# shanjiayao/PTT

Hardware: AMD Instinct MI355X
Metric: tracklet frames/sec (hot path: PointNet++ SA stack + Point-Track-Transformer blocks) (higher is better)
Workload: dtype f32

## Files before the change

### include/ptt_hip.h

```cpp
#ifndef PTT_HIP_H
#define PTT_HIP_H

#include <stddef.h>
#include <stdint.h>

#ifdef __cplusplus
extern "C" {
#endif

#define PTT_ABI_VERSION 28

enum {
    PTT_OK = 0,
    PTT_EINVAL = -1,
    PTT_EUNSUPPORTED = -2,
    PTT_ELAUNCH = -3,
    PTT_EWORKSPACE = -4
};

typedef void* ptt_stream_t;

int ptt_version(void);
const char* ptt_error_name(int code);
const char* ptt_last_error_string(void);

int ptt_fps_f32(const float* xyz, int B, int N, int npoint, int32_t* idx_out,
                ptt_stream_t stream);
int ptt_fps_ws_f32(const float* xyz, int B, int N, int npoint, int32_t* idx_out, float* workspace,
                   size_t workspace_elems, ptt_stream_t stream);

int ptt_gather_f32(const float* feat, const int32_t* idx, int B, int C, int N, int M,
                   float* out, ptt_stream_t stream);
int ptt_gather_grad_f32(const float* grad_out, const int32_t* idx, int B, int C, int N,
                        int M, float* grad_feat, ptt_stream_t stream);

int ptt_select_centres_f32(const float* xyz, const int32_t* idx, int B, int N, int M, float* new_xyz,
                           int64_t* idx64_out, ptt_stream_t stream);

int ptt_ball_query_f32(const float* new_xyz, const float* xyz, int B, int M, int N,
                       float radius, int nsample, int32_t* idx_out, ptt_stream_t stream);

int ptt_centres_ball_query_f32(const float* xyz, const int32_t* sel, int B, int N, int M, float radius, int nsample,
                               float* new_xyz, int64_t* idx64_out, int32_t* idx_out, ptt_stream_t stream);
// ... 476 lines not shown
```

### ptt_amd/csrc/common.h

```cpp
#pragma once
#include <hip/hip_runtime.h>
#include <stdint.h>
#include <stdio.h>
#include "../../include/ptt_hip.h"

namespace ptt {

char* last_error_buf();
int fail(int code, const char* fmt, ...);
int check_launch(const char* what);

static inline hipStream_t as_stream(ptt_stream_t s) { return reinterpret_cast<hipStream_t>(s); }

struct DevSwitches {
    int linear_rt = 1, linear_ct = 1;
    int linear_small = 1;
    int sa_gather1 = 0;
    int sa_stagger = 0;
    int sa_wave = 1;
    int sa_rt = 2;
    int sa_lds = 1;
    int sa_stream = 1;
    int sa_chunk = 2;
    int pair_stagger = 0;
    int pair_lds_pad = 0;
    int sa_lds_chunk = 2;
    int fps_plain = 0;
    int ball_cpw = 0;
    int fps_t = 0;
    int group_grad_global = 0;
    long long* stamps = nullptr;
};
const DevSwitches& dev_switches();

int set_lds_limit(const void* fn, int bytes);

bool wgrad_stream_ok(int R, int Cout, int Cin, int ldz, int ldx);
int wgrad_stream_rows(int R);
int launch_wgrad_stream(const float* dZ, int ldz, const float* X, int ldx, int R, int Cout, int Cin, int rows, float* partial,
                        const float* x_scale, const float* x_shift, hipStream_t s);

template <int CTRL, int ROW_MASK>
__device__ __forceinline__ int dpp_i32(int v) {
    return __builtin_amdgcn_update_dpp(v, v, CTRL, ROW_MASK, 0xF, false);
}
template <int CTRL, int ROW_MASK>
__device__ __forceinline__ float dpp_f32(float v) {
    return __builtin_bit_cast(float, dpp_i32<CTRL, ROW_MASK>(__builtin_bit_cast(int, v)));
}

__device__ __forceinline__ float wave_max_f32(float v) {
    v = fmaxf(v, dpp_f32<0xB1, 0xF>(v));
    v = fmaxf(v, dpp_f32<0x4E, 0xF>(v));
    v = fmaxf(v, dpp_f32<0x141, 0xF>(v));
    v = fmaxf(v, dpp_f32<0x140, 0xF>(v));
    v = fmaxf(v, dpp_f32<0x142, 0xA>(v));
    v = fmaxf(v, dpp_f32<0x143, 0xC>(v));
    return __builtin_bit_cast(float, __builtin_amdgcn_readlane(__builtin_bit_cast(int, v), 63));
}
__device__ __forceinline__ float wave_max_f32_fused(float v) {
    asm volatile(
        "s_nop 1\n\tv_max_f32_dpp %0, %0, %0 quad_perm:[1,0,3,2] row_mask:0xf bank_mask:0xf\n\t"
        "s_nop 1\n\tv_max_f32_dpp %0, %0, %0 quad_perm:[2,3,0,1] row_mask:0xf bank_mask:0xf\n\t"
        "s_nop 1\n\tv_max_f32_dpp %0, %0, %0 row_half_mirror row_mask:0xf bank_mask:0xf\n\t"
        "s_nop 1\n\tv_max_f32_dpp %0, %0, %0 row_mirror row_mask:0xf bank_mask:0xf\n\t"
        "s_nop 1\n\tv_max_f32_dpp %0, %0, %0 row_bcast:15 row_mask:0xa bank_mask:0xf\n\t"
        "s_nop 1\n\tv_max_f32_dpp %0, %0, %0 row_bcast:31 row_mask:0xc bank_mask:0xf\n\t"
        "s_nop 1"
// ... 25 lines not shown
```

### ptt_amd/csrc/gemm_ops.hip

```cpp
#include <atomic>
#include <math.h>
#include <stdlib.h>
#include <type_traits>
#include "common.h"

namespace ptt {

typedef float g32x16 __attribute__((ext_vector_type(16)));
typedef float g32x4 __attribute__((ext_vector_type(4)));
typedef int gi32x4 __attribute__((ext_vector_type(4)));
typedef unsigned int gu32x4 __attribute__((__vector_size__(4 * sizeof(unsigned int))));

namespace {

__device__ __forceinline__ __amdgpu_buffer_rsrc_t g_rsrc(const void* p) {
    return __builtin_amdgcn_make_buffer_rsrc(const_cast<void*>(p), 0, 0x7fffffff, 0x00020000);
}
__device__ __forceinline__ g32x4 g_load4(__amdgpu_buffer_rsrc_t r, int voff, int soff) {
    return __builtin_bit_cast(g32x4, __builtin_amdgcn_raw_buffer_load_b128(r, voff, soff, 0));
}
__device__ __forceinline__ float g_load1(__amdgpu_buffer_rsrc_t r, int voff, int soff) {
    return __builtin_bit_cast(float, __builtin_amdgcn_raw_buffer_load_b32(r, voff, soff, 0));
}
__device__ __forceinline__ void g_store1(float v, __amdgpu_buffer_rsrc_t r, int voff, int soff) {
// ... 469 lines not shown
        };
        frag(0, 0);
#pragma unroll
        for (int j = 0; j < RS / 2; ++j) {
            if (j + 1 < RS / 2) frag((EXP & 8) ? 0 : j + 1, (j + 1) & 1);
            __builtin_amdgcn_sched_barrier(0);
#pragma unroll
            for (int a = 0; a < TN; ++a)
#pragma unroll
                for (int b = 0; b < TK; ++b) acc[a][b] = __builtin_amdgcn_mfma_f32_32x32x2f32(av[j & 1][a], bv[j & 1][b], acc[a][b], 0, 0, 0);
            if (!(EXP & 1) && j >= RS / 2 - NP) stage_piece(buf ^ 1, j - (RS / 2 - NP));
            __builtin_amdgcn_sched_barrier(0);
        }
        if (!(EXP & 2)) hand_over();
        if (!(EXP & 4)) g_lds_barrier();
        buf ^= 1;
    }
    float* P = partial + (size_t)chunk * Cout * Cin;
#pragma unroll
    for (int a = 0; a < TN; ++a)
#pragma unroll
        for (int b = 0; b < TK; ++b) {
            const int ci = i0 + wk * (32 * TK) + b * 32 + col;
#pragma unroll
            for (int r = 0; r < 16; ++r) {
                const int co = o0 + wn * (32 * TN) + a * 32 + g_tile_row(r, half);
                if (!(EXP & 16) || r == 15) P[(size_t)co * Cin + ci] = acc[a][b][r];
            }
        }
}

void launch_wgrad_finish(const float* partial, int nchunks, size_t n, int accumulate, float* dW, hipStream_t s);

static int cu_count() {
    constexpr int MAX_DEV = 64;
    static std::atomic<int> cached[MAX_DEV];
    int dev = 0;
    if (hipGetDevice(&dev) != hipSuccess || dev < 0 || dev >= MAX_DEV) return 256;
    int n = cached[dev].load(std::memory_order_relaxed);
    if (n == 0) {
        int v = 0;
        n = (hipDeviceGetAttribute(&v, hipDeviceAttributeMultiprocessorCount, dev) == hipSuccess && v > 0) ? v : 256;
        cached[dev].store(n, std::memory_order_relaxed);
    }
    return n;
}

struct RowsGemmGeom { int WR, RT, CT, KC, TR, ncg, ntiles, G, chunks; bool ok; };
static RowsGemmGeom rows_gemm_geom(int rows, int K, int N) {
    RowsGemmGeom g{};
    g.ok = false;
    if (rows <= 0 || K <= 0 || N <= 0) return g;
    if (N % 128 == 0 && K % 128 == 0) {
        const int tiles64 = (rows + 63) / 64;
        g.WR = 1; g.RT = 2; g.KC = 128;
        g.CT = (N % 256 == 0 && (long long)tiles64 * (N / 256) >= 2 * cu_count()) ? 2 : 1;
    }
    else if (N % 128 == 0 && K % 64 == 0) { g.WR = 1; g.RT = 4; g.CT = 1; g.KC = 64; }
    else if (N % 64 == 0 && K % 64 == 0) { g.WR = 2; g.RT = 2; g.CT = 1; g.KC = 64; }
    else return g;
    const int WC = 4 / g.WR;
    g.TR = 32 * g.RT * g.WR;
    g.ncg = N / (32 * WC * g.CT);
    g.ntiles = (rows + g.TR - 1) / g.TR;
    int cap = 2 * cu_count() / g.ncg;
    if (cap >= 8) cap &= ~7;
    if (cap < 1) cap = 1;
// ... 378 lines not shown
```

### ptt_amd/csrc/mfma_ops.hip

```cpp
#include <math.h>
#include <stdlib.h>
#include <string.h>
#include "common.h"
#include "mfma_common.h"

#ifndef PTT_PAIR_PF
#define PTT_PAIR_PF 1
#endif
#ifndef PTT_GATHER_BATCH
#define PTT_GATHER_BATCH 16
#endif
#ifndef PTT_SA_WAVES
#define PTT_SA_WAVES 2
#endif

namespace ptt {

#ifdef PTT_DEV
#define PTT_STAMP(i) do { if (p.dbg && threadIdx.x == 0 && blockIdx.x < 4096) p.dbg[blockIdx.x * 8 + (i)] = __builtin_readcyclecounter(); } while (0)
#else
#define PTT_STAMP(i) do { } while (0)
#endif

__device__ __forceinline__ void stagger_second_slot(int first_wave_blocks, int quanta) {
// ... 1157 lines not shown
#pragma unroll
                    for (int r = 0; r < 16; ++r) acc[rt][u][r] = pre.sh[u];
            int nvalid = 0;
#pragma unroll
            for (int u = 0; u < 2; ++u)
                if (w + 4 * u < LL.NT) nvalid = u + 1;
            gemm_tiles<RT, 2, 0>(Xs, p.ldk, LL.nkb, reinterpret_cast<const f32x4*>(LL.Wp), LL.NT, w, nvalid, lane, acc, pre.w);
#pragma unroll
            for (int u = 0; u < 2; ++u) {
                if (u >= nvalid) break;
                const int col = (w + 4 * u) * 32 + (lane & 31);
                float sc = 1.f, sh = 0.f;
                if (affine) { sc = LL.scale[col]; sh = LL.shift ? LL.shift[col] : 0.f; }
#pragma unroll
                for (int rt = 0; rt < RT; ++rt) {
                    float m = affine ? acc[rt][u][0] * sc + sh : acc[rt][u][0];
#pragma unroll
                    for (int r = 1; r < 16; ++r) m = fmaxf(m, affine ? acc[rt][u][r] * sc + sh : acc[rt][u][r]);
                    run[u] = fmaxf(run[u], max_halves(m));
                }
            }
        }
    }
    if (half == 0) {
#pragma unroll
        for (int u = 0; u < 2; ++u) {
            if (w + 4 * u >= LL.NT) break;
            const int col = (w + 4 * u) * 32 + (lane & 31);
            p.out[(SPLIT ? hsel * q.out_sh : 0) + b * p.osb + col * p.osc + jj * p.osm] = LL.relu ? fmaxf(run[u], 0.f) : run[u];
        }
    }
}

template <int NS, int CT, bool AFFINE, int RT>
__device__ __forceinline__ void sa_wave_layer(const SaParams& p, const SaLayerDev& L, bool last, float* Xw, int lane,
                                              int centre0, int ncentres) {
    f32x16 acc[RT][CT];
#pragma unroll
    for (int u = 0; u < CT; ++u) {
        const float s0 = (!AFFINE && L.shift) ? L.shift[u * 32 + (lane & 31)] : 0.f;
#pragma unroll
        for (int rt = 0; rt < RT; ++rt)
#pragma unroll
            for (int r = 0; r < 16; ++r) acc[rt][u][r] = s0;
    }
    gemm_core<RT, CT, CT, 1>(Xw, p.ldk, L.nkb, reinterpret_cast<const f32x4*>(L.Wp), L.NT, 0, lane, acc);
    __builtin_amdgcn_wave_barrier();
    const int half = lane >> 5;
#pragma unroll
    for (int u = 0; u < CT; ++u) {
        const int col = u * 32 + (lane & 31);
        float sc = 1.f, sv = 0.f;
        if constexpr (AFFINE) { sc = L.scale[col]; sv = L.shift ? L.shift[col] : 0.f; }
#pragma unroll
        for (int rt = 0; rt < RT; ++rt) {
            float y[16];
#pragma unroll
            for (int r = 0; r < 16; ++r) y[r] = AFFINE ? acc[rt][u][r] * sc + sv : acc[rt][u][r];
            if (!last) {
#pragma unroll
                for (int r = 0; r < 16; ++r)
                    Xw[(rt * 32 + tile_row(r, half)) * p.ldk + col] = L.relu ? fmaxf(y[r], 0.f) : y[r];
            } else if (NS == 32) {
                float m = y[0];
#pragma unroll
                for (int r = 1; r < 16; ++r) m = fmaxf(m, y[r]);
// ... 943 lines not shown
        if ((rc = set_lds_limit(reinterpret_cast<const void*>(sa_stream_kernel<32>), lds))) return rc;
        hipLaunchKernelGGL((sa_stream_kernel<32>), dim3(wgs), dim3(256), lds, s, p);
        return check_launch("sa_stream_kernel");
    }
    int RT = dev_switches().sa_rt;
    if (d->nsample == 64) RT = 2;
    const int lds = 32 * RT * p.ldk * (int)sizeof(float);
    if (lds > 160 * 1024) return fail(PTT_EUNSUPPORTED, "ptt_sa_fused_fwd_f32: %d B of LDS per workgroup", lds);
    const int cpw = 32 * RT / d->nsample;
    const dim3 grid((total_centres + cpw - 1) / cpw);
#define PTT_SA_CASE(NSV, RTV)                                                                                   \
    if (d->nsample == NSV && RT == RTV) {                                                                       \
        if ((rc = set_lds_limit(reinterpret_cast<const void*>(sa_fused_kernel<NSV, RTV>), lds))) return rc;     \
        hipLaunchKernelGGL((sa_fused_kernel<NSV, RTV>), grid, dim3(256), lds, s, p);                            \
    }
    PTT_SA_CASE(32, 2) PTT_SA_CASE(32, 1) PTT_SA_CASE(16, 2) PTT_SA_CASE(16, 1) PTT_SA_CASE(64, 2)
#undef PTT_SA_CASE
    return check_launch("sa_fused_kernel");
}

extern "C" int ptt_xcorr_fused_fwd_f32(const ptt_xcorr_desc* d, ptt_stream_t stream) {
    if (!d) return fail(PTT_EINVAL, "ptt_xcorr_fused_fwd_f32: null descriptor");
    if (d->B < 0 || d->Ns <= 0 || d->C0 <= 0 || d->n_layers < 1 || d->n_layers > PTT_SA_MAX_LAYERS)
        return fail(PTT_EINVAL, "ptt_xcorr_fused_fwd_f32: B=%d Ns=%d C0=%d layers=%d", d->B, d->Ns, d->C0, d->n_layers);
    if (d->Nt <= 0 || (d->Nt % 64) != 0)
        return fail(PTT_EUNSUPPORTED, "ptt_xcorr_fused_fwd_f32: Nt=%d (the template seeds are walked in chunks of 64)", d->Nt);
    if (d->n_layers < 2) return fail(PTT_EUNSUPPORTED, "ptt_xcorr_fused_fwd_f32: needs at least two MFMA layers after layer 0");
    if ((d->C0 % 8) != 0 || d->C0 > 256) return fail(PTT_EUNSUPPORTED, "ptt_xcorr_fused_fwd_f32: C0=%d", d->C0);
    if (d->B == 0) return PTT_OK;
    if (!d->P || !d->w_sim || !d->out) return fail(PTT_EINVAL, "ptt_xcorr_fused_fwd_f32: null pointer");
    if ((unsigned long long)d->B * d->Ns * d->Nt >= 0x7fffffffull || (unsigned long long)d->B * d->Nt * d->C0 >= 0x7fffffffull)
        return fail(PTT_EUNSUPPORTED, "ptt_xcorr_fused_fwd_f32: B=%d Ns=%d Nt=%d: 32-bit element offsets — split the batch",
                    d->B, d->Ns, d->Nt);
    XcorrParams q;
    q.P = d->P; q.wsim = d->w_sim; q.scale0 = d->scale0;
    q.shift0 = d->shift0; q.sim_out = d->sim_out; q.cos_t = d->cos_t;
    q.C0 = d->C0; q.Nt = d->Nt;
    q.sfeat = q.tfeat = nullptr; q.s_sb = q.s_sn = q.t_sb = q.t_sn = 0; q.C = 0; q.eps = 0.f; q.out_sh = 0;
    SaParams& p = q.sa;
    memset(&p, 0, sizeof(p));
    p.out = d->out; p.osb = d->out_sb; p.osc = d->out_sc; p.osm = d->out_sn;
    p.B = d->B; p.M = d->Ns; p.n_layers = d->n_layers;
    int maxk = d->C0, cin = d->C0;
    for (int l = 0; l < d->n_layers; ++l) {
        const ptt_sa_layer& s = d->layers[l];
        if (s.Cin != cin) return fail(PTT_EINVAL, "ptt_xcorr_fused_fwd_f32: layer %d Cin=%d, expected %d", l, s.Cin, cin);
        if (s.Cout <= 0 || (s.Cout % 32) != 0 || s.Cout > 256)
            return fail(PTT_EUNSUPPORTED, "ptt_xcorr_fused_fwd_f32: layer %d Cout=%d", l, s.Cout);
        if (!s.Wpacked) return fail(PTT_EINVAL, "ptt_xcorr_fused_fwd_f32: layer %d has no weights", l);
        SaLayerDev& L = p.L[l];
        L.Wp = s.Wpacked; L.scale = s.scale; L.shift = s.shift; L.Cin = s.Cin; L.Cout = s.Cout; L.relu = s.relu;
        L.nkb = (s.Cin + 7) / 8; L.NT = s.Cout / 32;
        if (l + 1 < d->n_layers && s.Cout > maxk) maxk = s.Cout;
        cin = s.Cout;
    }
    p.ldk = ((maxk + 7) / 8) * 8 + 4;
    p.first_wave = 1024; p.stagger = 2;
    if (d->split) {
        if (!d->search_feat || !d->templ_feat || d->sim_out || (d->C & 3) || (d->s_sb & 3) || (d->s_sn & 3) ||
            (d->t_sb & 3) || (d->t_sn & 3) || ((reinterpret_cast<uintptr_t>(d->search_feat) | reinterpret_cast<uintptr_t>(d->templ_feat)) & 15) ||
            ((d->B * d->Ns) & 7) || d->C <= 0)
            return fail(PTT_EINVAL, "ptt_xcorr_fused_fwd_f32: the split form needs the features (unit channel stride, C %% 4 == 0, 16-byte "
                                    "aligned rows), B * Ns %% 8 == 0 and no sim_out");
        q.sfeat = d->search_feat; q.tfeat = d->templ_feat; q.s_sb = d->s_sb; q.s_sn = d->s_sn; q.t_sb = d->t_sb; q.t_sn = d->t_sn;
        q.C = d->C; q.eps = d->eps; q.out_sh = d->out_sh;
        const int lds = (32 * p.ldk + 32) * (int)sizeof(float);
        int rc = set_lds_limit(reinterpret_cast<const void*>(xcorr_fused_kernel<1, true>), lds);
        if (rc) return rc;
        hipLaunchKernelGGL((xcorr_fused_kernel<1, true>), dim3(2 * d->B * d->Ns), dim3(256), lds, as_stream(stream), q);
        return check_launch("xcorr_fused_kernel");
    }
    if (!d->cos_t) return fail(PTT_EINVAL, "ptt_xcorr_fused_fwd_f32: null pointer (cos_t comes from ptt_cosine_map_f32)");
    const int lds = (64 * p.ldk + 64) * (int)sizeof(float);
    int rc = set_lds_limit(reinterpret_cast<const void*>(xcorr_fused_kernel<2, false>), lds);
    if (rc) return rc;
    hipLaunchKernelGGL((xcorr_fused_kernel<2, false>), dim3(d->B * d->Ns), dim3(256), lds, as_stream(stream), q);
    return check_launch("xcorr_fused_kernel");
}

extern "C" int ptt_cosine_map_f32(const float* search_feat, int64_t s_sb, int64_t s_sn, int64_t s_sc, const float* templ_feat,
                                  int64_t t_sb, int64_t t_sn, int64_t t_sc, int B, int Ns, int Nt, int C, float eps,
                                  float* cos_t, ptt_stream_t stream) {
    if (B < 0 || Ns <= 0 || Nt <= 0 || C <= 0) return fail(PTT_EINVAL, "ptt_cosine_map_f32: B=%d Ns=%d Nt=%d C=%d", B, Ns, Nt, C);
    if (B == 0) return PTT_OK;
    if (!search_feat || !templ_feat || !cos_t) return fail(PTT_EINVAL, "ptt_cosine_map_f32: null pointer");
    CosParams q;
    q.sfeat = search_feat; q.tfeat = templ_feat; q.cos_t = cos_t;
    q.s_sb = s_sb; q.s_sn = s_sn; q.s_sc = s_sc; q.t_sb = t_sb; q.t_sn = t_sn; q.t_sc = t_sc;
    q.B = B; q.Ns = Ns; q.Nt = Nt; q.C = C; q.eps = eps;
    hipLaunchKernelGGL(cos_map_kernel, dim3((B * Ns + 3) / 4), dim3(256), 0, as_stream(stream), q);
// ... 45 lines not shown
```

### ptt_amd/models/backbones_3d/pointnet2_backbone.py

```python
from typing import List

import torch
import torch.nn as nn

from ... import graph_policy, ops, train_ops
from ...param_cache import ParamCache, index_table
from .pointnet2 import pointnet2_modules


class PointNet2BackboneLight(nn.Module):
    def __init__(self, model_cfg, input_channels, **kwargs):
        super().__init__()
        self.model_cfg = model_cfg
        input_channels -= 3
        self.num_points_each_layer = []
        self.SA_modules = nn.ModuleList()
        sa = self.model_cfg.SA_CONFIG
        for k in range(len(sa.RADIUS)):
            mlps = list(sa.MLPS[k])
            if k == 0:
                mlps[0] = input_channels
            self.SA_modules.append(pointnet2_modules.PointnetSAModuleVotes(
                radius=sa.RADIUS[k], nsample=sa.NSAMPLE[k], mlp=mlps,
                use_xyz=sa.get('USE_XYZ', True), normalize_xyz=sa.get('NORMALIZE_XYZ', True),
                sample_method=sa.SAMPLE_METHOD[k]))
        self.cov_final = nn.Conv1d(256, 256, kernel_size=1)
        self.num_point_features = sa.MLPS[-1][-1]
        self._cov_cache = ParamCache()
        self.seed_knn = 16
        self.overlap_branches = True
        self._side_stream = None

    @staticmethod
    def _break_up_pc(pc):
        xyz = pc[..., 0:3].contiguous()
        features = pc[..., 3:].contiguous() if pc.size(-1) > 3 else None
        return xyz, features

    def _cov_final(self, features):
        if not features.is_cuda:
            return self.cov_final(features)
        if self.training:
            if features.dtype != torch.float32:
                return self.cov_final(features)
            return train_ops.rows_linear(self.cov_final, features.transpose(1, 2)).transpose(1, 2)
        if ops.autograd_recording(self.cov_final, features) or features.dtype != torch.float32:
            ops.note_unfused('PointNet2BackboneLight.cov_final', 'autograd is recording or input is not float32')
            return self.cov_final(features)
        w, b = self.cov_final.weight, self.cov_final.bias
        wpacked, bias = self._cov_cache.get([w, b], w.device, lambda: (ops.pack_weight(w), b.detach().float().contiguous()))
        rows = features.transpose(1, 2)
        out = ops.linear(rows, wpacked, w.shape[0], None, bias)
        return out.transpose(1, 2)

    def branch_forward(self, pts, npoints: List, inds0=None, want_knn=0, compact_levels=()):
        xyz, features = self._break_up_pc(pts)
        sa = self.model_cfg.SA_CONFIG
        one_frame = (not self.training and xyz.is_cuda and features is None and len(self.SA_modules) == 3
                     and xyz.shape[0] * npoints[0] <= 4 * ops.ONE_FRAME_MAX_POINTS
                     and self.SA_modules[0].sample_method == 'fps'
                     and all(m.sample_method in ('rs', 'sequence') for m in self.SA_modules[1:])
                     and npoints[0] >= npoints[1] >= npoints[2] and (not want_knn or npoints[2] <= 128)
                     and all(m._fusable(xyz, None) for m in self.SA_modules[:1]))
        knn = None
# ... 6 lines not shown
            levels, inds64, knn = ops.sa_levels_point_jobs(xyz, inds0, list(npoints), list(sa.RADIUS), list(sa.NSAMPLE),
                                                           knn_k=want_knn)
            seq = [None] + [index_table(xyz.size(0), n, xyz.device, torch.int64) for n in npoints[1:3]]
            xyz, features, inds0 = self.SA_modules[0](xyz=xyz, features=features, npoint=npoints[0], inds=inds0,
                                                      pre=(levels[0][0], levels[0][1], inds64))
            xyz, features, inds1 = self.SA_modules[1](xyz=xyz, features=features, npoint=npoints[1],
                                                      pre=(levels[1][0], levels[1][1], seq[1]))
            xyz, features, inds2 = self.SA_modules[2](xyz=xyz, features=features, npoint=npoints[2],
                                                      pre=(levels[2][0], levels[2][1], seq[2]))
        else:
            xyz, features, inds0 = self.SA_modules[0](xyz=xyz, features=features, npoint=npoints[0], inds=inds0)
            xyz, features, inds1 = self.SA_modules[1](xyz=xyz, features=features, npoint=npoints[1], compact=1 in compact_levels)
            xyz, features, inds2 = self.SA_modules[2](xyz=xyz, features=features, npoint=npoints[2], compact=2 in compact_levels)
        point_features = self._cov_final(features)
        assert inds1.dtype == inds2.dtype == torch.int64, 'index type must be int64, not {}'.format(inds2.dtype)
        if all(m.sample_method in ('rs', 'sequence') for m in self.SA_modules[1:]) and inds0.shape[1] >= npoints[2]:
            inds = inds0[:, :npoints[2]]
        else:
            inds = inds0.gather(1, inds1).gather(1, inds2)
        if want_knn:
            return xyz, point_features, inds, knn
        return xyz, point_features, inds

    def sample(self, search_points, template_points):
        from .pointnet2 import pointnet2_utils
        sa = self.model_cfg.SA_CONFIG
        assert sa.SAMPLE_METHOD[0] == 'fps'
        return (pointnet2_utils.furthest_point_sample(search_points[..., 0:3].contiguous(), sa.NPOINTS_SEARCH[0]),
                pointnet2_utils.furthest_point_sample(template_points[..., 0:3].contiguous(), sa.NPOINTS_TEMPLATE[0]))

    def forward_branches(self, search_points, template_points, inds=None):
        sa = self.model_cfg.SA_CONFIG
        i_s, i_t = inds if inds is not None else (None, None)
        last = (len(self.SA_modules) - 1,) if (search_points.is_cuda and not self.training) else ()
        if not (self.overlap_branches and search_points.is_cuda and not self.training):
            r = self.branch_forward(search_points, sa.NPOINTS_SEARCH, i_s, want_knn=self.seed_knn, compact_levels=last)
            t_seeds, t_feats, t_inds = self.branch_forward(template_points, sa.NPOINTS_TEMPLATE, i_t)
        else:
            if self._side_stream is None or self._side_stream.device != search_points.device:
                self._side_stream = torch.cuda.Stream(device=search_points.device)
            main = torch.cuda.current_stream(search_points.device)
            side = graph_policy.branch(main, self._side_stream)
            with torch.cuda.stream(side):
                t_seeds, t_feats, t_inds = self.branch_forward(template_points, sa.NPOINTS_TEMPLATE, i_t)
            r = self.branch_forward(search_points, sa.NPOINTS_SEARCH, i_s, want_knn=self.seed_knn, compact_levels=last)
            graph_policy.join(main, side)
            if side is not main:
                for t in (t_seeds, t_feats, t_inds, template_points):
                    t.record_stream(main)
        s_seeds, s_feats, s_inds = r[:3]
        s_knn = r[3] if len(r) > 3 else None
        out = {'search_seeds': s_seeds, 'search_feats': s_feats, 'search_inds': s_inds,
               'template_seeds': t_seeds, 'template_feats': t_feats, 'template_inds': t_inds}
        if s_knn is not None:
            out['search_seeds_knn'] = s_knn
        return out

    def forward(self, batch_dict):
        batch_dict.update(self.forward_branches(batch_dict['search_points'], batch_dict['template_points'],
                                                batch_dict.pop('fps_inds', None)))
        batch_dict.pop('search_points')
        batch_dict.pop('template_points')
        return batch_dict
```

### ptt_amd/models/similarity_modules/p2b_xcoor.py

```python
import torch
import torch.nn as nn
import torch.nn.functional as F

from ... import ops, train_ops
from ...param_cache import DropsCachesOnModeChange, FoldedLayer, ParamCache, fold_conv_bn
from ..backbones_3d.pointnet2 import pytorch_utils as layer_utils


class CosineSimAug(DropsCachesOnModeChange, nn.Module):
    def __init__(self, model_cfg):
        super().__init__()
        self.model_cfg = model_cfg
        self.cosine = nn.CosineSimilarity(dim=1)
        self.mlp = layer_utils.SharedMLP(self.model_cfg.MLP.CHANNELS, bn=self.model_cfg.MLP.BN)
        self.conv = (
            layer_utils.Seq(self.model_cfg.CONV.CHANNELS[0])
            .conv1d(self.model_cfg.CONV.CHANNELS[1], bn=self.model_cfg.CONV.BN)
            .conv1d(self.model_cfg.CONV.CHANNELS[2], activation=None)
        )
        self._cache = ParamCache()

    def _fusable(self, search_feats, template_feats):
        if self.training or not search_feats.is_cuda:
            return False
        name = 'CosineSimAug'
        if ops.autograd_recording(self, search_feats, template_feats):
            return ops.note_unfused(name, 'autograd is recording (wrap inference in torch.no_grad())')
        if search_feats.dtype != torch.float32 or template_feats.dtype != torch.float32:
            return ops.note_unfused(name, 'features must be float32')
        if template_feats.shape[-1] % 64 != 0:
            return ops.note_unfused(name, 'ptt_xcorr_fused_fwd_f32 walks the template seeds in chunks of 64 (got %d)'
                                    % template_feats.shape[-1])
        units = list(self.mlp)
        if len(units) < 3 or len(units) > 5:
            return ops.note_unfused(name, 'SharedMLP depth %d' % len(units))
        for u in units:
            if not hasattr(u, 'normlayer') or u.conv.weight.shape[0] % 32 or u.conv.weight.shape[0] > 256:
                return ops.note_unfused(name, 'SharedMLP needs BatchNorm and widths that are multiples of 32, <= 256')
        if len(self.conv) != 2 or not hasattr(self.conv[0], 'normlayer') or hasattr(self.conv[1], 'normlayer'):
# ... 12 lines not shown
        s0, t0 = fold_conv_bn(units[0])
        layers = []
        for u in units[1:]:
            sc, sh = fold_conv_bn(u)
            w = u.conv.weight
            layers.append(FoldedLayer(ops.pack_weight(w * sc.view(-1, 1, 1, 1)), None, sh, w.shape[1], w.shape[0], True))
        return dict(w_sim=(w0[:, 0].float() * s0).contiguous(), w_rest=ops.pack_weight(w0[:, 1:]), c0=w0.shape[0],
                    w_rest_fx=ops.pack_weight(w0[:, 1:], 3),
                    scale0=s0, shift0=t0, layers=layers)

    def forward(self, batch_dict):
        search_feats = batch_dict['search_feats']
        template_feats = batch_dict['template_feats']
        template_xyz = batch_dict['template_seeds']
        b, f, n2 = search_feats.shape
        n1 = template_feats.shape[-1]

        if self._fusable(search_feats, template_feats):
            P = self._params()
            trows = template_feats.transpose(1, 2)
            if b * n1 <= ops.ONE_FRAME_MAX_POINTS and trows.is_contiguous():
                pre = torch.empty((b, n1, P['c0']), dtype=torch.float32, device=trows.device)
                ops.row_jobs([ops.row_job(P['w_rest_fx'], P['c0'], x=trows, x2=template_xyz.contiguous(), scale=P['scale0'],
                                          shift=P['shift0'], out=pre)])
            else:
                rows = torch.cat((template_xyz, trows), dim=2)
                pre = ops.linear(rows, P['w_rest'], P['c0'], P['scale0'], P['shift0'])
            if b * n2 <= ops.ONE_FRAME_MAX_POINTS:
                fused, _ = ops.xcorr_fused(search_feats, template_feats, pre, P['w_sim'], None, None,
                                           P['layers'], eps=self.cosine.eps, split=True)
            else:
                cos_t = ops.cosine_map(search_feats, template_feats, eps=self.cosine.eps)
                fused, _ = ops.xcorr_fused(search_feats, template_feats, pre, P['w_sim'], None, None,
                                           P['layers'], eps=self.cosine.eps, cos_t=cos_t)
            if fused.dim() == 4:
                L = layer_utils.rows_layers(self.conv)
                h0, h1 = fused[0].transpose(1, 2), fused[1].transpose(1, 2)
                x = None
                for li, layer in enumerate(L):
                    y = torch.empty((b, n2, layer.cout), dtype=torch.float32, device=h0.device)
                    ops.row_jobs([layer_utils.layer_job(layer, x=h0 if li == 0 else x, xmax=h1 if li == 0 else None, out=y)])
                    x = y
            else:
                y = layer_utils.rows_forward(self.conv, fused.transpose(1, 2))
            batch_dict['cosine_feats'] = y.transpose(1, 2)
            return batch_dict

        if (train_ops.usable(self.mlp, search_feats) and self.mlp[0].conv.weight.shape[1] == f + 4
                and self.mlp[0].conv.weight.shape[0] % 4 == 0 and self.mlp[0].conv.weight.shape[0] <= 256):
            fused = train_ops.xcorr_hoisted(search_feats, template_feats, template_xyz, self.mlp, self.cosine.eps)
            if train_ops.conv1d_stack_usable(self.conv, fused):
                batch_dict['cosine_feats'] = train_ops.conv1d_stack_rows(self.conv, fused.transpose(1, 2)).transpose(1, 2)
            else:
                batch_dict['cosine_feats'] = self.conv(fused)
            return batch_dict
        sim_feat = self.cosine(template_feats.unsqueeze(-1).expand(b, f, n1, n2),
                               search_feats.unsqueeze(2).expand(b, f, n1, n2))
        template_xyz_ = template_xyz.transpose(1, 2).contiguous().unsqueeze(-1).expand(b, 3, n1, n2)
        fusion_feature = torch.cat((sim_feat.unsqueeze(1), template_xyz_), dim=1)
        fusion_feature = torch.cat((fusion_feature, template_feats.unsqueeze(-1).expand(b, f, n1, n2)), dim=1)
        if train_ops.usable(self.mlp, fusion_feature):
            batch_dict['cosine_feats'] = self.conv(train_ops.shared_mlp_pool(fusion_feature, self.mlp, pool_dim=2))
            return batch_dict
        fusion_feature = self.mlp(fusion_feature)
        fusion_feature = fusion_feature.max(dim=2)[0]
        batch_dict['cosine_feats'] = self.conv(fusion_feature)
        return batch_dict
# ... 1 lines not shown
```

### ptt_amd/models/trackers/tracker3d_template.py

```python
import os

import torch
import torch.nn as nn

from .. import backbones_3d, similarity_modules, voting_heads


class Tracker3DTemplate(nn.Module):
    def __init__(self, model_cfg, num_class, dataset):
        super().__init__()
        self.model_cfg = model_cfg
        self.num_class = num_class
        self.dataset = dataset
        self.training = dataset.training
        self.class_names = dataset.class_names
        self.register_buffer('global_step', torch.LongTensor(1).zero_())
        self.module_topology = ['backbone_3d', 'similarity_module', 'centroid_voting_head', 'box_voting_head']

    @property
    def mode(self):
        return 'TRAIN' if self.training else 'TEST'

    def forward(self, **kwargs):
        raise NotImplementedError

    def update_global_step(self):
        self.global_step += 1

    def build_networks(self):
        info = {
            'module_list': [],
            'num_rawpoint_features': self.dataset.point_feature_encoder.num_point_features,
            'num_point_features': self.dataset.point_feature_encoder.num_point_features,
            'grid_size': self.dataset.grid_size,
            'point_cloud_range': self.dataset.point_cloud_range,
            'voxel_size': self.dataset.voxel_size,
        }
        for name in self.module_topology:
            module, info = getattr(self, 'build_%s' % name)(model_info_dict=info)
            self.add_module(name, module)
        return info['module_list']

    def build_backbone_3d(self, model_info_dict):
        cfg = self.model_cfg.get('BACKBONE_3D', None)
        if cfg is None:
            return None, model_info_dict
        module = backbones_3d.__all__[cfg.NAME](
            model_cfg=cfg, input_channels=model_info_dict['num_point_features'],
            grid_size=model_info_dict['grid_size'], voxel_size=model_info_dict['voxel_size'],
            point_cloud_range=model_info_dict['point_cloud_range'])
        model_info_dict['module_list'].append(module)
        model_info_dict['num_point_features'] = module.num_point_features
        return module, model_info_dict

    def build_similarity_module(self, model_info_dict):
        cfg = self.model_cfg.get('SIMILARITY_MODULE', None)
        if cfg is None:
            return None, model_info_dict
        module = similarity_modules.__all__[cfg.NAME](model_cfg=cfg)
        model_info_dict['module_list'].append(module)
        return module, model_info_dict

    def _build_head(self, key, model_info_dict):
        cfg = self.model_cfg.get(key, None)
        if cfg is None:
            return None, model_info_dict
        module = voting_heads.__all__[cfg.NAME](
            model_cfg=cfg, input_channels=model_info_dict['num_point_features'], num_class=1)
        model_info_dict['module_list'].append(module)
        return module, model_info_dict

    def build_centroid_voting_head(self, model_info_dict):
        return self._build_head('CENTROID_HEAD', model_info_dict)

    def build_box_voting_head(self, model_info_dict):
        return self._build_head('BOX_HEAD', model_info_dict)

    def post_processing(self, batch_dict):
        pass

    def load_params_from_file(self, filename, logger, to_cpu=False):
        if not os.path.isfile(filename):
            raise FileNotFoundError(filename)
# ... 34 lines not shown
```

### ptt_amd/ops.py

```python
import contextlib
import ctypes
import os

import torch

from . import _lib
from ._lib import AttnDesc, SaDesc, SaLayer, XcorrDesc


def _stream():
    return ctypes.c_void_p(torch.cuda.current_stream().cuda_stream)


_timing = None


def start_kernel_timing(names):
    global _timing
    _timing = {n: [] for n in names}


def stop_kernel_timing():
    global _timing
    t, _timing = _timing, None
# ... 384 lines not shown
    out = torch.empty((B, Ns, Nt), dtype=torch.float32, device=search_feats.device)
    ssb, ssc, ssn = search_feats.stride()
    tsb, tsc, tsn = templ_feats.stride()
    _launch("ptt_cosine_map_f32", out.device, search_feats.data_ptr(), ssb, ssn, ssc, templ_feats.data_ptr(), tsb, tsn, tsc, B, Ns, Nt, C, float(eps),
            out.data_ptr(), timed='ptt_cosine_map_f32')
    return out


def rows_mlp(x, layers, residual=None):
    if not x.is_cuda or x.dtype != torch.float32 or x.stride(-1) != 1:
        raise RuntimeError("rows_mlp: x must be a float32 device tensor with contiguous rows")
    K = x.shape[-1]
    x2 = x.reshape(-1, K)
    rows = x2.shape[0]
    cout = int(layers[-1][4])
    out = torch.empty((rows, cout), dtype=torch.float32, device=x.device)
    res2 = None
    if residual is not None:
        res2 = residual.reshape(-1, cout)
        _chk(res2 if res2.is_contiguous() else res2.contiguous(), "residual", torch.float32, 2)
        res2 = res2 if res2.stride(1) == 1 else res2.contiguous()
    arr = (SaLayer * len(layers))()
    for i, (wp, sc, sh, cin, co, relu) in enumerate(layers):
        arr[i].Wpacked = wp.data_ptr()
        arr[i].scale = sc.data_ptr() if sc is not None else None
        arr[i].shift = sh.data_ptr() if sh is not None else None
        arr[i].Cin, arr[i].Cout, arr[i].relu = int(cin), int(co), int(bool(relu))
    _launch("ptt_rows_mlp_f32", x.device, _ptr(x2), rows, K, x2.stride(0), arr, len(layers), _ptr(res2), res2.stride(0) if res2 is not None else 0,
            _ptr(out), cout, timed='ptt_rows_mlp_f32')
    return out.view(*x.shape[:-1], cout)


def xcorr_fused(search_feats, templ_feats, P, w_sim, scale0, shift0, layers, eps=1e-8, want_sim=False, cos_t=None, split=False):
    for t_, n_ in ((search_feats, "search_feats"), (templ_feats, "templ_feats")):
        if not t_.is_cuda or t_.dtype != torch.float32 or t_.dim() != 3:
            raise RuntimeError("%s must be a (B,C,N) float32 device tensor" % n_)
    _chk(P, "P", torch.float32, 3)
    _chk(w_sim, "w_sim", torch.float32, 1)
    B, C, Ns = search_feats.shape
    Nt = templ_feats.shape[2]
    C0 = P.shape[2]
    if Nt <= 0 or Nt % 64:
        raise RuntimeError("xcorr_fused: Nt=%d (ptt_xcorr_fused_fwd_f32 walks the template seeds in chunks of 64)" % Nt)
    if P.shape[0] != B or P.shape[1] != Nt or w_sim.shape[0] != C0 or templ_feats.shape[:2] != search_feats.shape[:2]:
        raise RuntimeError("xcorr_fused: inconsistent shapes")
    cout = layers[-1][4]
    split = (split and not want_sim and search_feats.stride(1) == 1 and templ_feats.stride(1) == 1 and C % 4 == 0 and (B * Ns) % 8 == 0
             and all(st % 4 == 0 for st in (search_feats.stride(0), search_feats.stride(2), templ_feats.stride(0), templ_feats.stride(2)))
             and search_feats.data_ptr() % 16 == 0 and templ_feats.data_ptr() % 16 == 0 and bool(layers[-1][5]))
    if not split:
        if cos_t is None:
            cos_t = cosine_map(search_feats, templ_feats, eps=eps)
        _chk(cos_t, "cos_t", torch.float32, 3)
        if tuple(cos_t.shape) != (B, Ns, Nt):
            raise RuntimeError("xcorr_fused: cos_t must be (B,Ns,Nt)")
    store = torch.empty(((2, B, Ns, cout) if split else (B, Ns, cout)), dtype=torch.float32, device=P.device)
    out = store.transpose(-1, -2)
    sim = torch.empty((B, Nt, Ns), dtype=torch.float32, device=P.device) if want_sim else None
    d = XcorrDesc()
    if split:
        d.split, d.out_sh = 1, store.stride(0)
        d.search_feat, d.templ_feat = search_feats.data_ptr(), templ_feats.data_ptr()
        d.s_sb, d.s_sn, d.t_sb, d.t_sn = search_feats.stride(0), search_feats.stride(2), templ_feats.stride(0), templ_feats.stride(2)
        d.C, d.eps = int(C), float(eps)
    else:
        d.cos_t = cos_t.data_ptr()
    d.P, d.w_sim = P.data_ptr(), w_sim.data_ptr()
    d.scale0 = scale0.data_ptr() if scale0 is not None else None
    d.shift0 = shift0.data_ptr() if shift0 is not None else None
    d.out = out.data_ptr()
    d.out_sb, d.out_sc, d.out_sn = out.stride()[-3:]
    d.sim_out = sim.data_ptr() if sim is not None else None
    d.B, d.Ns, d.Nt, d.C0 = B, Ns, Nt, C0
    d.n_layers = len(layers)
    for i, (wp, sc, sh, cin, co, relu) in enumerate(layers):
        L = d.layers[i]
        L.Wpacked = wp.data_ptr()
        L.scale = sc.data_ptr() if sc is not None else None
        L.shift = sh.data_ptr() if sh is not None else None
        L.Cin, L.Cout, L.relu = int(cin), int(co), int(bool(relu))
    _launch("ptt_xcorr_fused_fwd_f32", P.device, ctypes.byref(d), timed='ptt_xcorr_fused_fwd_f32')
    return out, sim


def pack_delta0(weight, bias):
    return pack_weight(torch.cat([weight.detach().float().reshape(weight.shape[0], 3),
                                  bias.detach().float().reshape(-1, 1)], dim=1).contiguous())


def spatial_order(xyz):
    _chk(xyz, "xyz", torch.float32, 3)
    B, N, _ = xyz.shape
    order = torch.empty((B, N), dtype=torch.int32, device=xyz.device)
    _launch("ptt_spatial_order_f32", xyz.device, _ptr(xyz), B, N, _ptr(order))
    return order


def pt_attn_pair(xyz, knn_idx, qkv, wd1p, wd2p, bd2, wg1p, bg1, wg2p, bg2, d_model, want_attn=True, rel=None, order=None,
                 heads=1):
# ... 1232 lines not shown
```

Measured before the change: 17430.

## Add persistent streamed xcorr kernel and compact more backbone SA levels

Adds a persistent kernel for the xcorr head that handles Nt=64, C0=256 with two 256-wide layers. For each search point it builds the first-layer activations from cos_t and the precomputed P in LDS, runs both layers with MFMA, and max-reduces over template seeds without writing intermediates. The grid is sized to two blocks per CU, and each block loops over a contiguous range of points, reusing P per batch and prefetching weights. The backbone also enables compact levels 1 and 2 for the search and template branches. The costs are added code paths with strict shape gating, and a behaviour change in SA level handling that could shift the balance of work.

```diff
diff --git a/include/ptt_hip.h b/include/ptt_hip.h
--- a/include/ptt_hip.h
+++ b/include/ptt_hip.h
@@ -8,7 +8,7 @@
 extern "C" {
 #endif
 
-#define PTT_ABI_VERSION 28
+#define PTT_ABI_VERSION 29
 
 enum {
     PTT_OK = 0,
diff --git a/ptt_amd/csrc/common.h b/ptt_amd/csrc/common.h
--- a/ptt_amd/csrc/common.h
+++ b/ptt_amd/csrc/common.h
@@ -34,6 +34,8 @@
 const DevSwitches& dev_switches();
 
 int set_lds_limit(const void* fn, int bytes);
+
+int cu_count();
 
 bool wgrad_stream_ok(int R, int Cout, int Cin, int ldz, int ldx);
 int wgrad_stream_rows(int R);
diff --git a/ptt_amd/csrc/gemm_ops.hip b/ptt_amd/csrc/gemm_ops.hip
--- a/ptt_amd/csrc/gemm_ops.hip
+++ b/ptt_amd/csrc/gemm_ops.hip
@@ -525,7 +525,7 @@
 
 void launch_wgrad_finish(const float* partial, int nchunks, size_t n, int accumulate, float* dW, hipStream_t s);
 
-static int cu_count() {
+int cu_count() {
     constexpr int MAX_DEV = 64;
     static std::atomic<int> cached[MAX_DEV];
     int dev = 0;
diff --git a/ptt_amd/csrc/mfma_ops.hip b/ptt_amd/csrc/mfma_ops.hip
--- a/ptt_amd/csrc/mfma_ops.hip
+++ b/ptt_amd/csrc/mfma_ops.hip
@@ -1213,6 +1213,115 @@
     }
 }
 
+constexpr int XCS_C = 256;
+constexpr int XCS_LDK = XCS_C + 4;
+constexpr int XCS_NKB = XCS_C / 8, XCS_NT = XCS_C / 32;
+__global__ __launch_bounds__(256, 2) void xcorr_stream_kernel(XcorrParams q) {
+    typedef float f32x2 __attribute__((ext_vector_type(2)));
+    extern __shared__ __attribute__((aligned(16))) float smem[];
+    float* Xs = smem;
+    const SaParams& p = q.sa;
+    const int t = threadIdx.x, lane = t & 63, w = __builtin_amdgcn_readfirstlane(t >> 6), half = lane >> 5;
+    const int npts = p.B * p.M;
+    const int g = logical_block(), G = (int)gridDim.x;
+    const int base = npts / G, rem = npts - base * G;
+    int j = g * base + min(g, rem);
+    const int jend = j + base + (g < rem ? 1 : 0);
+    if (j >= jend) return;
+    stagger_second_slot(p.first_wave, p.stagger);
+
+    const SaLayerDev& L0 = p.L[0];
+    const SaLayerDev& L1 = p.L[1];
+    const f32x4* W0 = reinterpret_cast<const f32x4*>(L0.Wp);
+    const f32x4* W1 = reinterpret_cast<const f32x4*>(L1.Wp);
+    const int col0 = w * 32 + (lane & 31);
+    const float sh0[2] = {L0.shift[col0], L0.shift[col0 + 128]};
+    const float sh1[2] = {L1.shift[col0], L1.shift[col0 + 128]};
+    const f32x4 w4 = *reinterpret_cast<const f32x4*>(q.wsim + lane * 4);
+    const int crow = w + 4 * (lane & 15);
+
+    int b = j / p.M;
+    const int pvoff = (w * XCS_C + lane * 4) * (int)sizeof(float);
+    f32x4 pq[16];
+    {
+        const __amdgpu_buffer_rsrc_t pr = weight_rsrc(q.P + (size_t)b * (64 * XCS_C));
+#pragma unroll
+        for (int k = 0; k < 16; ++k) pq[k] = weight_load(pr, pvoff, k * 4 * XCS_C * (int)sizeof(float));
+    }
+    float cv = q.cos_t[(unsigned)(j * 64 + crow)];
+    f32x4 pre[2];
+    prefetch_first_block_full<2>(L0.Wp, w, lane, pre);
+
+    for (;;) {
+#pragma unroll
+        for (int k = 0; k < 16; ++k) {
+            const float cs = __builtin_bit_cast(float, __builtin_amdgcn_readlane(__builtin_bit_cast(int, cv), k));
+            const f32x2 c2 = {cs, cs};
+            const f32x4 pv = pq[k];
+            f32x2 lo = __builtin_elementwise_fma(f32x2{w4[0], w4[1]}, c2, f32x2{pv[0], pv[1]});
+            f32x2 hi = __builtin_elementwise_fma(f32x2{w4[2], w4[3]}, c2, f32x2{pv[2], pv[3]});
+            *reinterpret_cast<f32x4*>(Xs + (w + 4 * k) * XCS_LDK + lane * 4) =
+                f32x4{fmaxf(lo[0], 0.f), fmaxf(lo[1], 0.f), fmaxf(hi[0], 0.f), fmaxf(hi[1], 0.f)};
+        }
+        lds_barrier();
+
+        f32x16 acc[2][2];
+#pragma unroll
+        for (int rt = 0; rt < 2; ++rt)
+#pragma unroll
+            for (int u = 0; u < 2; ++u)
+#pragma unroll
+                for (int r = 0; r < 16; ++r) acc[rt][u][r] = sh0[u];
+        gemm_core<2, 2, 2, 4, 0>(Xs, XCS_LDK, XCS_NKB, W0, XCS_NT, w, lane, acc, pre);
+        prefetch_first_block_full<2>(L1.Wp, w, lane, pre);
+        lds_barrier();
+#pragma unroll
+        for (int u = 0; u < 2; ++u)
+#pragma unroll
+            for (int rt = 0; rt < 2; ++rt)
+#pragma unroll
+                for (int r = 0; r < 16; ++r)
+                    Xs[(rt * 32 + tile_row(r, half)) * XCS_LDK + col0 + u * 128] = L0.relu ? fmaxf(acc[rt][u][r], 0.f) : acc[rt][u][r];
+        lds_barrier();
+
+        const int jn = j + 1;
+        const bool more = jn < jend;
+        const int jl = more ? jn : j;
+        const int bn = jl / p.M;
+        cv = q.cos_t[(unsigned)(jl * 64 + crow)];
+        if (bn != b) {
+            const __amdgpu_buffer_rsrc_t pr = weight_rsrc(q.P + (size_t)bn * (64 * XCS_C));
+#pragma unroll
+            for (int k = 0; k < 16; ++k) pq[k] = weight_load(pr, pvoff, k * 4 * XCS_C * (int)sizeof(float));
+        }
+
+#pragma unroll
+        for (int rt = 0; rt < 2; ++rt)
+#pragma unroll
+            for (int u = 0; u < 2; ++u)
+#pragma unroll
+                for (int r = 0; r < 16; ++r) acc[rt][u][r] = sh1[u];
+        gemm_core<2, 2, 2, 4, 0>(Xs, XCS_LDK, XCS_NKB, W1, XCS_NT, w, lane, acc, pre);
+        prefetch_first_block_full<2>(L0.Wp, w, lane, pre);
+        const int jj = j - b * p.M;
+#pragma unroll
+        for (int u = 0; u < 2; ++u) {
+            float run = -__builtin_inff();
+#pragma unroll
+            for (int rt = 0; rt < 2; ++rt) {
+                float m = acc[rt][u][0];
+#pragma unroll
+                for (int r = 1; r < 16; ++r) m = fmaxf(m, acc[rt][u][r]);
+                run = fmaxf(run, max_halves(m));
+            }
+            if (half == 0) p.out[b * p.osb + (col0 + u * 128) * p.osc + jj * p.osm] = L1.relu ? fmaxf(run, 0.f) : run;
+        }
+        if (!more) break;
+        j = jn; b = bn;
+        lds_barrier();
+    }
+}
+
 template <int NS, int CT, bool AFFINE, int RT>
 __device__ __forceinline__ void sa_wave_layer(const SaParams& p, const SaLayerDev& L, bool last, float* Xw, int lane,
                                               int centre0, int ncentres) {
@@ -2222,6 +2331,22 @@
     if ((unsigned long long)d->B * d->Ns * d->Nt >= 0x7fffffffull || (unsigned long long)d->B * d->Nt * d->C0 >= 0x7fffffffull)
         return fail(PTT_EUNSUPPORTED, "ptt_xcorr_fused_fwd_f32: B=%d Ns=%d Nt=%d: 32-bit element offsets — split the batch",
                     d->B, d->Ns, d->Nt);
+    const bool streamed = d->split == 2;
+    if (streamed) {
+        if (!d->cos_t) return fail(PTT_EUNSUPPORTED, "ptt_xcorr_fused_fwd_f32: the streamed form reads cos_t (ptt_cosine_map_f32)");
+        if (d->Nt != 64 || d->C0 != XCS_C || d->n_layers != 2)
+            return fail(PTT_EUNSUPPORTED, "ptt_xcorr_fused_fwd_f32: the streamed form is Nt=64, C0=256 and two remaining layers (Nt=%d C0=%d layers=%d)",
+                        d->Nt, d->C0, d->n_layers);
+        if (d->scale0 || d->shift0) return fail(PTT_EUNSUPPORTED, "ptt_xcorr_fused_fwd_f32: the streamed form needs layer 0's BatchNorm folded into P and w_sim");
+        if (d->sim_out) return fail(PTT_EUNSUPPORTED, "ptt_xcorr_fused_fwd_f32: the streamed form does not write sim_out");
+        for (int l = 0; l < 2; ++l) {
+            const ptt_sa_layer& s = d->layers[l];
+            if (s.Cin != XCS_C || s.Cout != XCS_C)
+                return fail(PTT_EUNSUPPORTED, "ptt_xcorr_fused_fwd_f32: the streamed form is 256 -> 256 -> 256 (layer %d: %d -> %d)", l, s.Cin, s.Cout);
+            if (s.scale || !s.shift)
+                return fail(PTT_EUNSUPPORTED, "ptt_xcorr_fused_fwd_f32: the streamed form needs layer %d's scale folded into its weights and a shift", l);
+        }
+    }
     XcorrParams q;
     q.P = d->P; q.wsim = d->w_sim; q.scale0 = d->scale0;
     q.shift0 = d->shift0; q.sim_out = d->sim_out; q.cos_t = d->cos_t;
@@ -2246,6 +2371,14 @@
     }
     p.ldk = ((maxk + 7) / 8) * 8 + 4;
     p.first_wave = 1024; p.stagger = 2;
+    if (streamed) {
+        const int npts = d->B * d->Ns, slots = 2 * cu_count();
+        const int lds = 64 * XCS_LDK * (int)sizeof(float);
+        int rc = set_lds_limit(reinterpret_cast<const void*>(xcorr_stream_kernel), lds);
+        if (rc) return rc;
+        hipLaunchKernelGGL(xcorr_stream_kernel, dim3(npts < slots ? npts : slots), dim3(256), lds, as_stream(stream), q);
+        return check_launch("xcorr_stream_kernel");
+    }
     if (d->split) {
         if (!d->search_feat || !d->templ_feat || d->sim_out || (d->C & 3) || (d->s_sb & 3) || (d->s_sn & 3) ||
             (d->t_sb & 3) || (d->t_sn & 3) || ((reinterpret_cast<uintptr_t>(d->search_feat) | reinterpret_cast<uintptr_t>(d->templ_feat)) & 15) ||
diff --git a/ptt_amd/models/backbones_3d/pointnet2_backbone.py b/ptt_amd/models/backbones_3d/pointnet2_backbone.py
--- a/ptt_amd/models/backbones_3d/pointnet2_backbone.py
+++ b/ptt_amd/models/backbones_3d/pointnet2_backbone.py
@@ -30,6 +30,8 @@
         self.seed_knn = 16
         self.overlap_branches = True
         self._side_stream = None
+        self.compact_levels = (len(self.SA_modules) - 1,)
+        self.template_compact_levels = ()
 
     @staticmethod
     def _break_up_pc(pc):
@@ -102,17 +104,19 @@
     def forward_branches(self, search_points, template_points, inds=None):
         sa = self.model_cfg.SA_CONFIG
         i_s, i_t = inds if inds is not None else (None, None)
-        last = (len(self.SA_modules) - 1,) if (search_points.is_cuda and not self.training) else ()
+        fused = search_points.is_cuda and not self.training
+        last = tuple(self.compact_levels) if fused else ()
+        t_levels = tuple(self.template_compact_levels) if fused else ()
         if not (self.overlap_branches and search_points.is_cuda and not self.training):
             r = self.branch_forward(search_points, sa.NPOINTS_SEARCH, i_s, want_knn=self.seed_knn, compact_levels=last)
-            t_seeds, t_feats, t_inds = self.branch_forward(template_points, sa.NPOINTS_TEMPLATE, i_t)
+            t_seeds, t_feats, t_inds = self.branch_forward(template_points, sa.NPOINTS_TEMPLATE, i_t, compact_levels=t_levels)
         else:
             if self._side_stream is None or self._side_stream.device != search_points.device:
                 self._side_stream = torch.cuda.Stream(device=search_points.device)
             main = torch.cuda.current_stream(search_points.device)
             side = graph_policy.branch(main, self._side_stream)
             with torch.cuda.stream(side):
-                t_seeds, t_feats, t_inds = self.branch_forward(template_points, sa.NPOINTS_TEMPLATE, i_t)
+                t_seeds, t_feats, t_inds = self.branch_forward(template_points, sa.NPOINTS_TEMPLATE, i_t, compact_levels=t_levels)
             r = self.branch_forward(search_points, sa.NPOINTS_SEARCH, i_s, want_knn=self.seed_knn, compact_levels=last)
             graph_policy.join(main, side)
             if side is not main:
diff --git a/ptt_amd/models/similarity_modules/p2b_xcoor.py b/ptt_amd/models/similarity_modules/p2b_xcoor.py
--- a/ptt_amd/models/similarity_modules/p2b_xcoor.py
+++ b/ptt_amd/models/similarity_modules/p2b_xcoor.py
@@ -5,6 +5,9 @@
 from ... import ops, train_ops
 from ...param_cache import DropsCachesOnModeChange, FoldedLayer, ParamCache, fold_conv_bn
 from ..backbones_3d.pointnet2 import pytorch_utils as layer_utils
+
+
+XCORR_STREAM_MIN_POINTS = 512
 
 
 class CosineSimAug(DropsCachesOnModeChange, nn.Module):
@@ -83,7 +86,8 @@
             else:
                 cos_t = ops.cosine_map(search_feats, template_feats, eps=self.cosine.eps)
                 fused, _ = ops.xcorr_fused(search_feats, template_feats, pre, P['w_sim'], None, None,
-                                           P['layers'], eps=self.cosine.eps, cos_t=cos_t)
+                                           P['layers'], eps=self.cosine.eps, cos_t=cos_t,
+                                           split=2 if b * n2 >= XCORR_STREAM_MIN_POINTS else False)
             if fused.dim() == 4:
                 L = layer_utils.rows_layers(self.conv)
                 h0, h1 = fused[0].transpose(1, 2), fused[1].transpose(1, 2)
diff --git a/ptt_amd/models/trackers/tracker3d_template.py b/ptt_amd/models/trackers/tracker3d_template.py
--- a/ptt_amd/models/trackers/tracker3d_template.py
+++ b/ptt_amd/models/trackers/tracker3d_template.py
@@ -49,6 +49,8 @@
             model_cfg=cfg, input_channels=model_info_dict['num_point_features'],
             grid_size=model_info_dict['grid_size'], voxel_size=model_info_dict['voxel_size'],
             point_cloud_range=model_info_dict['point_cloud_range'])
+        if hasattr(module, 'compact_levels'):
+            module.compact_levels = module.template_compact_levels = (1, 2)
         model_info_dict['module_list'].append(module)
         model_info_dict['num_point_features'] = module.num_point_features
         return module, model_info_dict
diff --git a/ptt_amd/ops.py b/ptt_amd/ops.py
--- a/ptt_amd/ops.py
+++ b/ptt_amd/ops.py
@@ -440,6 +440,9 @@
 
 
 def xcorr_fused(search_feats, templ_feats, P, w_sim, scale0, shift0, layers, eps=1e-8, want_sim=False, cos_t=None, split=False):
+    streamed = split == 2 and not isinstance(split, bool)
+    if streamed:
+        split = False
     for t_, n_ in ((search_feats, "search_feats"), (templ_feats, "templ_feats")):
         if not t_.is_cuda or t_.dtype != torch.float32 or t_.dim() != 3:
             raise RuntimeError("%s must be a (B,C,N) float32 device tensor" % n_)
@@ -456,6 +459,8 @@
     split = (split and not want_sim and search_feats.stride(1) == 1 and templ_feats.stride(1) == 1 and C % 4 == 0 and (B * Ns) % 8 == 0
              and all(st % 4 == 0 for st in (search_feats.stride(0), search_feats.stride(2), templ_feats.stride(0), templ_feats.stride(2)))
              and search_feats.data_ptr() % 16 == 0 and templ_feats.data_ptr() % 16 == 0 and bool(layers[-1][5]))
+    streamed = (streamed and not want_sim and Nt == 64 and C0 == 256 and scale0 is None and shift0 is None and len(layers) == 2
+                and all(sc is None and sh is not None and cin == 256 and co == 256 for (_, sc, sh, cin, co, _) in layers))
     if not split:
         if cos_t is None:
             cos_t = cosine_map(search_feats, templ_feats, eps=eps)
@@ -473,6 +478,7 @@
         d.C, d.eps = int(C), float(eps)
     else:
         d.cos_t = cos_t.data_ptr()
+        d.split = 2 if streamed else 0
     d.P, d.w_sim = P.data_ptr(), w_sim.data_ptr()
     d.scale0 = scale0.data_ptr() if scale0 is not None else None
     d.shift0 = shift0.data_ptr() if shift0 is not None else None
```

Result: no change. 17370 (-0.3%).
